# User-tian/Conan

Hardware: AMD Instinct MI355X
Metric: chunks/sec (80 ms chunk, 16 kHz), all streams summed; p50 per-chunk latency beside it (higher is better)
Workload: dtype f32 (3×bf16-limb products, f32 accumulate)

## Files before the change

### conan_amd/csrc/kernels.h

```cpp
#pragma once
#include <hip/hip_runtime.h>
#include <stdint.h>
#include <stdlib.h>

#include "voice_layout.h"

namespace cnk {

inline const char* dev_getenv(const char* name) {
#ifdef CONAN_DEV_SWITCHES
  return getenv(name);
#else
  (void)name;
  return nullptr;
#endif
}
#define HIP_CHECK(x) ::ch::hip_check((x), #x)


struct TRef {
  float* base;
  long long slot_stride;
  int C;
  int lmask;
// ... 101 lines not shown
  const int* tiles;
  const int* assign;
  int assign_per;
  int wr_max;
  float* slab; int* counters;
  long long slab_floats; int max_counters;
};
bool conv_limb_supported(const ConvArgs& a);
int conv_limb_shape(const ConvArgs* p, int nprob, int num_cu, int plan_n = 0, bool tail_split = false);
bool launch_conv_limb(const ConvLimbGroup& g, int shape, int num_cu, hipStream_t st);
int conv_limb_tail_slices(const ConvArgs& a, int shape, int num_cu);
const char* conv_limb_name(int shape);

struct RBProb {
  const float* w1; const float* w2;
  const float* b1; const float* b2;
  const unsigned short* w1l; const unsigned short* w2l;
  TRef x;
  TRef y;
  int k, dil;
};
struct RBArgs {
  RBProb p[3];
  const int* slots; const int* pos;
  const int* tiles;
  int ntiles;
  int* sched;
  int nprob, n, T;
  int tiles_per_slot;
  int order[3];
  float slope;
  int merge;
  TRef ymean;
  unsigned long long* dbg;
};
bool resblock_fused_supported(int C, int kmax, int span_max);
int resblock_fused_rows(int C, int T, int n, int ksum, int kmax, int num_cu);
bool launch_resblock_fused(const RBArgs& a, int C, int rows, int num_cu, hipStream_t st);
bool resblock_fused_can_merge(int C, int rows);
const char* resblock_fused_name(int C, int rows, bool merge = false);
const int* resblock_tiles(const RBArgs& a, int ro, int* total_out);
bool resblock_limb_supported(int C, int kmax, int span_max);
constexpr int kResblockLimbMaxSlots = 256;
int resblock_limb_rows(int C, int span_max);
bool launch_resblock_limb(const RBArgs& a, int C, int rows, int num_cu, hipStream_t st);
bool resblock_limb_can_merge(int C, int rows);
const char* resblock_limb_name(int C, int rows, bool merge = false);


struct RPProb {
  const float* w1; const float* w2;
  const float* b1; const float* b2;
  TRef x, y;
  TRef xh;
  int k, dil;
};
struct RPArgs {
  RPProb p[3];
  const int* slots; const int* pos;
  const int* tiles; int ntiles;
  int* sched;
  float* xb;
  unsigned* xflag; unsigned* mbox; unsigned* xcount;
  int nprob, n, T;
  float slope;
  unsigned* guard;
// ... 415 lines not shown
```

### conan_amd/csrc/resblock_limb.hip

```cpp
#include <algorithm>
#include <cstring>
#include <type_traits>

#include "kernels.h"

#define RL_MAX_SLOTS 256

#ifndef RL_HELPER_PRIO
#define RL_HELPER_PRIO 3
#endif
#ifndef RL_MATRIX_PRIO
#define RL_MATRIX_PRIO 0
#endif
#ifndef RL_STAMPS
#define RL_STAMPS 0
#endif

#ifdef RL_ABLATE_W
#define RL_WOFF(x) 0
#define RL_WOFF2(a_, b_) (b_)
#else
#define RL_WOFF(x) (x)
#define RL_WOFF2(a_, b_) (a_)
#endif

namespace cnk {

namespace {

typedef float f32x4 __attribute__((ext_vector_type(4)));
typedef __bf16 bf16x8 __attribute__((ext_vector_type(8)));
typedef unsigned short u16;
typedef const f32x4 __attribute__((address_space(1)))* gcf4;
typedef f32x4 __attribute__((address_space(1)))* gf4;
typedef const float __attribute__((address_space(1)))* gcf1;
typedef const int __attribute__((address_space(1)))* gci;

__device__ __forceinline__ f32x4 rl_gload(const void* p) { return *(gcf4)(p); }
__device__ __forceinline__ float4 rl_gload4(const float* p) { const f32x4 v = *(gcf4)(p); return make_float4(v[0], v[1], v[2], v[3]); }
__device__ __forceinline__ void rl_gstore4(float* p, const float4 v) { *(gf4)(p) = (f32x4){v.x, v.y, v.z, v.w}; }

typedef float f32x2 __attribute__((ext_vector_type(2)));
typedef __bf16 bf16x2 __attribute__((ext_vector_type(2)));
__device__ __forceinline__ void rl_split2(const f32x2 x, unsigned& h, unsigned& m, unsigned& l) {
  h = __builtin_bit_cast(unsigned, __builtin_convertvector(x, bf16x2));
  const f32x2 hf = {__uint_as_float(h << 16), __uint_as_float(h & 0xffff0000u)};
  const f32x2 r1 = x - hf;
  m = __builtin_bit_cast(unsigned, __builtin_convertvector(r1, bf16x2));
  const f32x2 mf = {__uint_as_float(m << 16), __uint_as_float(m & 0xffff0000u)};
  const f32x2 r2 = r1 - mf;
  l = __builtin_bit_cast(unsigned, __builtin_convertvector(r2, bf16x2));
}
__device__ __forceinline__ f32x2 rl_lrelu2(const f32x2 x, const float slope) {
  const f32x2 sx = x * slope;
  return (f32x2){__builtin_fmaxf(x[0], sx[0]), __builtin_fmaxf(x[1], sx[1])};
}

template <int C_, int NR2_, int SPAN_>
struct RLGeom {
  static constexpr int C = C_, NR2 = NR2_;
  static constexpr int NR1 = NR2 + 1;
  static constexpr int RO = 16 * NR2;
  static constexpr int XT_ROWS = 16 * NR1;
  static constexpr int MAXSPAN = SPAN_;
  static constexpr int WR_MAX = XT_ROWS + MAXSPAN;
  static constexpr int LDB = C + 16;
  static constexpr int PLW = WR_MAX * LDB;
  static constexpr int PLX = XT_ROWS * LDB;
  static constexpr int LDA = C + 4;
  static constexpr int LDS_U16 = 3 * (PLW + PLX);
  static constexpr int NCT = C / 16;
  static constexpr int NCW = C == 64 ? 1 : 2;
  static constexpr int RSPLIT = 4 / (NCT / NCW);
// ... 181 lines not shown
        const int idx = ht + 256 * u;
        const int w = idx / G::C4, c4 = idx - w * G::C4;
        const unsigned row = (rbase + (unsigned)w) & rmask;
        wv[u] = idx < wtotal ? rl_gload4(xb + (long long)row * C + c4 * 4) : make_float4(0.f, 0.f, 0.f, 0.f);
      }
      const long long abs0 = (xmode == 0 ? (long long)pos * xrate : 0ll) + t0 - (k - 1);
      wzr = abs0 >= 0 ? 0 : (abs0 < -(long long)G::XT_ROWS ? G::XT_ROWS : (int)-abs0);
    };
    auto win_write = [&]() __attribute__((always_inline)) {
#pragma unroll
      for (int u = 0; u < NIT; ++u) {
        const int idx = ht + 256 * u;
        const int w = idx / G::C4, c4 = idx - w * G::C4;
        unsigned h[2], m[2], l[2];
        rl_split2(rl_lrelu2((f32x2){wv[u].x, wv[u].y}, slope), h[0], m[0], l[0]);
        rl_split2(rl_lrelu2((f32x2){wv[u].z, wv[u].w}, slope), h[1], m[1], l[1]);
        if (idx < wtotal) {
          u16* dst = win + w * LDB + c4 * 4;
          *reinterpret_cast<uint2*>(dst) = make_uint2(h[0], h[1]);
          *reinterpret_cast<uint2*>(dst + G::PLW) = make_uint2(m[0], m[1]);
          *reinterpret_cast<uint2*>(dst + 2 * G::PLW) = make_uint2(l[0], l[1]);
        }
      }
      if (ht == 0) meta[0] = wzr;
    };
    constexpr int NOUT = (G::RO * G::C4) / 256;
    static_assert((G::RO * G::C4) % 256 == 0 && 256 % G::C4 == 0, "output tile / helper threads");
    const int oc4 = ht % G::C4;
    float4 oacc[NOUT], ores[NOUT], osum[MERGE ? NOUT : 1], ob2 = make_float4(0.f, 0.f, 0.f, 0.f);
    const float* oxb = nullptr; const float* ob2p = nullptr;
    float* oyb = nullptr;
    unsigned oyr0 = 0, oym = 0, oxr0 = 0, oxm = 0;
    int ot0 = 0, op = 0, oyC = C;
#pragma unroll
    for (int u = 0; u < (MERGE ? NOUT : 1); ++u) osum[u] = make_float4(0.f, 0.f, 0.f, 0.f);
    auto out_fetch = [&](const int p, const int i, const int t0, const int slot, const int pos) __attribute__((always_inline)) {
      const int xmode = a.p[0].x.mode, xrate = a.p[0].x.rate, ymode = a.p[0].y.mode, yrate = a.p[0].y.rate;
      oxb = RL_SEL(p, x.base) + (long long)(xmode == 0 ? slot : i) * RL_SEL(p, x.slot_stride);
      oxr0 = (xmode == 0 ? (unsigned)pos * (unsigned)xrate : 0u) + (unsigned)(RL_SEL(p, x.off) + t0);
      oxm = xmode == 0 ? (unsigned)RL_SEL(p, x.lmask) : 0xffffffffu;
      if (!merge) {
        oyb = RL_SEL(p, y.base) + (long long)(ymode == 0 ? slot : i) * RL_SEL(p, y.slot_stride);
        oyr0 = (ymode == 0 ? (unsigned)pos * (unsigned)yrate : 0u) + (unsigned)(RL_SEL(p, y.off) + t0);
        oym = ymode == 0 ? (unsigned)RL_SEL(p, y.lmask) : 0xffffffffu;
      } else {
        const int mmode = a.ymean.mode;
        oyb = a.ymean.base + (long long)(mmode == 0 ? slot : i) * a.ymean.slot_stride;
        oyr0 = (mmode == 0 ? (unsigned)pos * (unsigned)a.ymean.rate : 0u) + (unsigned)(a.ymean.off + t0);
        oym = mmode == 0 ? (unsigned)a.ymean.lmask : 0xffffffffu;
        oyC = a.ymean.C;
      }
      ot0 = t0; op = p;
      ob2p = RL_SEL(p, b2) + oc4 * 4;
#pragma unroll
      for (int u = 0; u < NOUT; ++u) oacc[u] = *reinterpret_cast<const float4*>(accimg + ((ht + 256 * u) / G::C4) * G::LDA + oc4 * 4);
      ob2 = rl_gload4(ob2p);
#pragma unroll
      for (int u = 0; u < NOUT; ++u) {
        const int r = (ht + 256 * u) / G::C4;
        ores[u] = ot0 + r < T ? rl_gload4(oxb + (long long)((oxr0 + (unsigned)r) & oxm) * C + oc4 * 4) : make_float4(0.f, 0.f, 0.f, 0.f);
      }
    };
    auto out_store = [&]() __attribute__((always_inline)) {
#pragma unroll
      for (int u = 0; u < NOUT; ++u) {
        const int r = (ht + 256 * u) / G::C4;
        if (ot0 + r < T) {
          const float4 v = make_float4((oacc[u].x + ob2.x) + ores[u].x, (oacc[u].y + ob2.y) + ores[u].y, (oacc[u].z + ob2.z) + ores[u].z, (oacc[u].w + ob2.w) + ores[u].w);
          if constexpr (!MERGE) rl_gstore4(oyb + (long long)((oyr0 + (unsigned)r) & oym) * C + oc4 * 4, v);
          else {
            float4 sm = osum[MERGE ? u : 0];
            if (op == 0) sm = v; else { sm.x += v.x; sm.y += v.y; sm.z += v.z; sm.w += v.w; }
            osum[MERGE ? u : 0] = sm;
            if (op == np - 1) {
              const float dn = (float)np;
              if (np > 1) { sm.x /= dn; sm.y /= dn; sm.z /= dn; sm.w /= dn; }
              sm.x = sm.x > 0.f ? sm.x : sm.x * slope; sm.y = sm.y > 0.f ? sm.y : sm.y * slope;
              sm.z = sm.z > 0.f ? sm.z : sm.z * slope; sm.w = sm.w > 0.f ? sm.w : sm.w * slope;
              rl_gstore4(oyb + (long long)((oyr0 + (unsigned)r) & oym) * oyC + oc4 * 4, sm);
            }
          }
        }
      }
    };
#if RL_STAMPS
    const unsigned long long h_t0 = __builtin_amdgcn_s_memtime();
    unsigned long long h_t[6] = {0, 0, 0, 0, 0, 0};
#define RL_HT(i_) h_t[i_] = __builtin_amdgcn_s_memtime() - h_t0
#else
#define RL_HT(i_)
#endif
    int dv0 = 0;
    if (wave == 4 && lane == 0) dv0 = __hip_atomic_fetch_add(a.sched, 1, __ATOMIC_RELAXED, __HIP_MEMORY_SCOPE_AGENT);
    for (int e = ht; e < a.n; e += 256) {
      const int sl = a.slots ? *(gci)(a.slots + e) : e;
      sptab[2 * e] = sl; sptab[2 * e + 1] = a.pos ? *(gci)(a.pos + sl) : 0;
    }
    const int tps = a.tiles_per_slot, per_prob = a.n * tps;
    auto decode = [&](const int e, int& p, int& i, int& t0) __attribute__((always_inline)) {
      if constexpr (!MERGE) {
        const int b = e / per_prob, rem = e - b * per_prob;
        p = b == 0 ? a.order[0] : (b == 1 ? a.order[1] : a.order[2]);
        i = rem / tps; t0 = (rem - i * tps) * G::RO;
      } else {
        const int g = e / np;
        p = e - g * np; i = g / tps; t0 = (g - i * tps) * G::RO;
      }
    };
    int cur = -1, p = -1, i = 0, t0 = 0;
    if (wave == 4) {
      cur = __builtin_amdgcn_readfirstlane(dv0) * (merge ? np : 1);
      if (cur >= ntiles) cur = -1;
      if (cur >= 0) decode(cur, p, i, t0);
      if (lane == 0) { meta[1] = cur; meta[2] = p; meta[3] = 0; }
    }
    RL_HT(0);
// ... 224 lines not shown
#endif
}


namespace {
struct RLCand { int C, NR2, span; };
const RLCand kLimbCands[] = {{32, 10, 50}, {64, 5, 50}, {128, 2, 50}};
}

bool resblock_limb_supported(int C, int kmax, int span_max) {
  for (const RLCand& c : kLimbCands)
    if (c.C == C && span_max <= c.span) return kmax <= 16;
  return false;
}

int resblock_limb_rows(int C, int span_max) {
  int best = 0;
  for (const RLCand& c : kLimbCands)
    if (c.C == C && span_max <= c.span) best = std::max(best, 16 * c.NR2);
  return best;
}

template <int C, int NR2, int SPAN, bool MERGE = false>
static bool launch_rl(const RBArgs& ain, int num_cu, hipStream_t st) {
  RBArgs a = ain;
  const int ro = 16 * NR2;
  a.tiles_per_slot = (a.T + ro - 1) / ro;
  const int total = a.nprob * a.n * a.tiles_per_slot;
  if (total <= 0) return true;
  if (!a.sched) return false;
  for (int p = 0; p < a.nprob; ++p) if (!a.p[p].w1l || !a.p[p].w2l) return false;
  if (a.n > RL_MAX_SLOTS) return false;
  if (!(a.slope > 0.f && a.slope <= 1.f)) return false;
  for (int p = 0; p < 3; ++p) a.order[p] = p;
  std::stable_sort(a.order, a.order + a.nprob, [&](int x, int y) { return a.p[x].k > a.p[y].k; });
  const int grid = std::min(a.merge ? total / a.nprob : total, num_cu);
  a.tiles = nullptr; a.ntiles = total;
  hipLaunchKernelGGL((resblock_limb_kernel<C, NR2, SPAN, MERGE>), dim3(grid), dim3(512), 0, st, a);
  return true;
}

bool launch_resblock_limb(const RBArgs& a, int C, int rows, int num_cu, hipStream_t st) {
  const int nr2 = rows / 16;
  if (a.merge) {
    if (C == 32 && nr2 == 10) return launch_rl<32, 10, 50, true>(a, num_cu, st);
    if (C == 64 && nr2 == 5) return launch_rl<64, 5, 50, true>(a, num_cu, st);
    if (C == 128 && nr2 == 2) return launch_rl<128, 2, 50, true>(a, num_cu, st);
    return false;
  }
  if (C == 32 && nr2 == 10) return launch_rl<32, 10, 50>(a, num_cu, st);
  if (C == 64 && nr2 == 5) return launch_rl<64, 5, 50>(a, num_cu, st);
  if (C == 128 && nr2 == 2) return launch_rl<128, 2, 50>(a, num_cu, st);
  return false;
}

bool resblock_limb_can_merge(int C, int rows) { return (C == 32 && rows == 160) || (C == 64 && rows == 80) || (C == 128 && rows == 32); }

const char* resblock_limb_name(int C, int rows, bool merge) {
  static thread_local char buf[72];
  const int span = 50;
  snprintf(buf, sizeof(buf), "cnk::resblock_limb_kernel<%d, %d, %d, %s>", C, rows / 16, span, merge ? "true" : "false");
  return buf;
}

}
```

### conan_amd/csrc/streams.h

```cpp
#pragma once
#include <array>
#include <functional>

#include "host_common.h"
#include "snapshot_layout.h"
#include "voice_layout.h"

using ch::Error;
using ch::Lin;
using ch::PackedConv;
using ch::Ring;
using cnk::ConvArgs;
using cnk::ConvGroup;
using cnk::TRef;

constexpr int kMaxBranches = 3;
constexpr int PADR = 16;

struct VocStage {
  Ring up;
  Ring upa;
  Ring xs;
  std::vector<std::vector<Ring>> xt, xo;
  std::vector<std::vector<Ring>> xa;
// ... 69 lines not shown
      auto it = dev_plan.find(name);
      if (it != dev_plan.end()) return it->second.c_str();
    }
#ifdef CONAN_DEV_SWITCHES
    return getenv((std::string("CONAN_") + name).c_str());
#else
    return nullptr;
#endif
  }
  bool fixed_plan = false;
  bool in_style_pass = false;
  int plan_n(int n) const { return (fixed_plan && !in_style_pass) ? max_slots : n; }
  bool pipe_idle = false;
  bool shared_device = false;
  int max_slots = 0, max_frames = 0, max_ref = 0, S_max = 0;
  std::vector<void*> allocs;
  int64_t state_bytes = 0;
  std::vector<std::pair<float*, long long>> voc_state, dec_state, emf_state;

  int* d_slots = nullptr;
  int* d_ident = nullptr;
  int* d_zero = nullptr;
  int* d_lens = nullptr;
  int* d_lens2 = nullptr;
  int* d_codes = nullptr;
  float* sk_slab[3] = {nullptr, nullptr, nullptr};
  int* sk_counters[3] = {nullptr, nullptr, nullptr};
  int reserve_cus = 0;
  bool fenced = false;
  bool rb_limb = false;
  bool arith_auto = true;
  bool rb_merge = true;
  int* cp_ticket[3] = {nullptr, nullptr, nullptr};
  int* rb_sched[2] = {nullptr, nullptr};
  float* rp_xb[2] = {nullptr, nullptr};
  unsigned* rp_words[2] = {nullptr, nullptr};
  long long sk_slab_floats = 0;
  int sk_max_tiles = 0;
  std::vector<int> h_slots;
  std::vector<int> slot_seen;
  int slot_gen = 0;
  PinRing pin;
  int* pos_emf = nullptr; int* pos_dec = nullptr; int* pos_voc = nullptr;
  unsigned* d_guard = nullptr;
  unsigned* h_guard = nullptr;
  int test_fault = 0;
  void check_fault() const {
    if (!h_guard) return;
    const unsigned code = *(volatile const unsigned*)h_guard;
    if (code == 0) return;
    static const char* what[] = {"?", "decoder_mega_kernel group / grid barrier", "emformer_fused_kernel cluster exchange", "resblock_pair_kernel partner flag", "resblock_pair_kernel tile mailbox",
                                 "(retired)", "decoder_mega_kernel xcd election", "decoder_mega_kernel xcd roll call", "decoder_mega_kernel xcd flag barrier"};
    throw ch::Error(CONAN_ERR_HIP, std::string("a cross-workgroup wait gave up after its 50 ms budget (") + what[code < 9 ? code : 0] +
                                       "): results since then are invalid and this stream-set is unusable - destroy it and create a new one");
  }

  struct FeSlot { long long recv = 0; int frames = 0, chunks = 0, phase = 0; };
  struct RsSlot { const ch::RsTable* f = nullptr; long long in = 0, out = 0; int phase = 0; };
  struct WavIn {
    float* fe_audio = nullptr; float* fe_mel = nullptr; float* fe_chunk = nullptr;
    int fe_LA = 0, fe_LM = 0, fe_last_n = 0;
    std::vector<FeSlot> fe_slot;
    StageSets<RgRow> rg_sets;
    int* rg_codes[kStageSets] = {}; float* rg_mel[kStageSets] = {}; float* rg_wav[kStageSets] = {};
    bool fe_last_ragged = false;
    std::vector<RsSlot> rs_slot;
// ... 129 lines not shown

  void mega_print_stamps();
  ~conan_streams() {
    if (live) live->fetch_sub(1);
    if (mega_dbg) mega_print_stamps();
    if (st_emf) (void)hipStreamDestroy(st_emf);
    if (st_front) (void)hipStreamDestroy(st_front);
    if (st_voc) (void)hipStreamDestroy(st_voc);
    for (int i = 0; i < NP; ++i) { if (ev_in[i]) (void)hipEventDestroy(ev_in[i]); if (ev_fence[i]) (void)hipEventDestroy(ev_fence[i]); }
    for (int i = 0; i < NP; ++i) { if (ev_wide[i]) (void)hipEventDestroy(ev_wide[i]); if (ev_emf[i]) (void)hipEventDestroy(ev_emf[i]); if (ev_front[i]) (void)hipEventDestroy(ev_front[i]); if (ev_voc[i]) (void)hipEventDestroy(ev_voc[i]); }
    for (void* p : allocs) (void)hipFree(p);
    if (h_guard) (void)hipHostFree(h_guard);
    for (auto& e : prof_ev) { (void)hipEventDestroy(e.first); (void)hipEventDestroy(e.second); }
    for (auto& e : clock_ev) (void)hipEventDestroy(e);
    for (auto& m : mega_cache) { if (m.copied) (void)hipEventDestroy(m.copied); if (m.pinned) (void)hipHostFree(m.pinned); if (m.dev) (void)hipFree(m.dev); }
    for (auto& e : tl_ev) (void)hipEventDestroy(e);
  }

  void build_vocoder();
  void build_emformer();
  void build_decoder();
  void set_slots(const int32_t* slots, int n, hipStream_t st);
  int pick_cfg(int M, int N, int nprob) const;
  bool prof_on = false;
  std::vector<std::pair<hipEvent_t, hipEvent_t>> prof_ev;
  size_t prof_used = 0;
  double prof_flops = 0.0;
  long long prof_launches = 0;
  struct ProfRec { std::string name; double flops; };
  std::vector<ProfRec> prof_rec;
  struct ProfKernel { std::string name; double ms, flops; long long n; };
  std::vector<ProfKernel> prof_kernels;
  void launch_group(const ConvGroup& g, int nprob, int cfg, hipStream_t st);
  bool launch_rb(const cnk::RBArgs& a, int C, hipStream_t st, const TRef* ymean = nullptr);
  void launch_rp(const cnk::RPArgs& a, hipStream_t st);
  bool use_rowconv = true;
  bool rowconv_ok(const PackedConv& pc, int dil, int T) const { return use_rowconv && pc.wf && cnk::rowconv_supported(pc.Cin, pc.k, dil, T); }
  cnk::RowConvArgs mk_rc(const PackedConv& pc, const TRef& x, const TRef& y, int n, int T, int dil = 1) const;
  void rowconv(const cnk::RowConvArgs& a, hipStream_t st);
  template <typename F> void profiled(const std::string& name, double flops, hipStream_t st, F&& launch);
  void conv(const ConvArgs& a, hipStream_t st) { ConvGroup g; g.p[0] = a; launch_group(g, 1, pick_cfg(plan_n(a.n) * a.T, a.Cout, 1), st); }
  ConvArgs mk(const PackedConv& pc, const TRef& x, const TRef& y, int n, int T, const int* pos, int dil = 1, int pad_left = -1) const;

  struct DecExtra { float* mel_out2 = nullptr; int* codes_dst = nullptr; const int* codes_src = nullptr; int codes_words = 0;
                    const float* f0_in = nullptr; const float* uv_in = nullptr; };
  struct MegaProgram {
    long long key[8] = {0, 0, 0, 0, 0, 0, 0, 0};
    bool ok = false;
    int nops = 0, groups = 0, group_size = 0, njobs = 0, kw4 = 0, lds_bytes = 0, barriers = 0, n = 0, T = 0;
    int lds_need = 0;
    bool xcd = false;
    double flops = 0.0;
    cnk::MegaOp* dev = nullptr;
    cnk::MegaOp* pinned = nullptr;
    hipEvent_t copied = nullptr;
    long long stamp = 0;
  };
  static constexpr int kMegaMaxOps = cnk::kMegaMaxOps, kMegaEntries = 12;
  std::vector<MegaProgram> mega_cache;
  long long mega_clock = 0;
  bool use_mega = true;
  int mega_grid = 128;
  int mega_gs = 8;
  bool mega_narrow_ksplit = true;
  int mega_ffn_gs = 8;
  unsigned* mega_bar = nullptr;
  unsigned mega_bar_count = 0;
// ... 107 lines not shown
```

### conan_amd/csrc/streams.hip

```cpp
#include <climits>

#include "streams.h"


ConvArgs conan_streams::mk(const PackedConv& pc, const TRef& x, const TRef& y, int n, int T, const int* pos, int dil,
                           int pad_left) const {
  ConvArgs a;
  memset(&a, 0, sizeof(a));
  a.x = x;
  a.y = y; a.res = ch::null_ref(); a.m1 = ch::null_ref(); a.m2 = ch::null_ref();
  a.w = pc.w; a.bias = pc.bias; a.bvec = nullptr; a.slots = d_slots; a.pos = pos; a.lens = nullptr;
  a.Cin = pc.Cin; a.Cin_pad = pc.Cin_pad; a.Cin_alloc = pc.Cin_alloc; a.Cout = pc.Cout; a.Cout_pad = pc.Cout_pad;
  a.ktaps = pc.k; a.dil = dil; a.pad_left = pad_left < 0 ? (pc.k - 1) * dil : pad_left;
  a.T = T; a.n = n; a.in_act = cnk::ACT_NONE; a.in_slope = 0.f; a.out_act = cnk::ACT_NONE; a.out_scale = 1.f; a.out_slope = 0.f;
  a.shuffle_r = pc.shuffle_r;
  a.wl = reinterpret_cast<const unsigned short*>(pc.wl);
  if (x.C != pc.Cin && !(x.C > pc.Cin)) throw Error(CONAN_ERR_SHAPE, "conv input width mismatch");
  return a;
}

int conan_streams::pick_cfg(int M, int N, int nprob) const {
  const int wide[] = {cnk::CFG_64x64, cnk::CFG_32x64_K2, cnk::CFG_32x32_K4};
  const int narrow[] = {cnk::CFG_128x32, cnk::CFG_64x32_K2, cnk::CFG_32x32_K4};
  const int* order = N <= 32 ? narrow : wide;
// ... 112 lines not shown
void conan_streams::rowconv(const cnk::RowConvArgs& a, hipStream_t st) {
  const double fl = 2.0 * (double)a.n * a.T * a.Cout * a.ktaps * a.Cin;
  if (mega_rec) {
    cnk::MegaOp op; memset(&op, 0, sizeof(op));
    op.u.rc = a;
    int ldsf = 0;
    const int prows = fixed_plan ? plan_n(a.n) * a.T : 0;
    const int v = cnk::rowconv_plan(op.u.rc, &op.nbx, &op.nby, &ldsf, prows);
    op.type = v == 3 ? cnk::MOP_ROWLIN : (v == 2 ? cnk::MOP_RC114 : cnk::MOP_RC111);
    const int strips64 = (op.u.rc.Cout_pad + 63) / 64;
    if (v == 0 && !a.w2 && plan_n(a.n) * a.T > 16 && mega_narrow_ksplit && (strips64 * 4 <= mega_gs || (strips64 * 2 <= mega_gs && a.ktaps >= 3)) && (a.ktaps * (a.Cin >> 4)) % 4 == 0) {
      const int ldsk = (32 + op.u.rc.wr_max * (a.Cin + 8) + 3 * 64 * 4);
      cnk::MegaOp t = op; t.type = cnk::MOP_RC114;
      if (cnk::decoder_mega_lds_floats(t, ldsk) * 4 <= (96 + 32 * 264) * 4) {
        op.type = cnk::MOP_RC114; op.nbx = (op.u.rc.Cout_pad + 15) / 16; ldsf = ldsk;
      }
    }
    if (a.w2) {
      if ((v != 0 && v != 2) || (a.ktaps * (a.Cin >> 4)) % 8 != 0) { mega_rec_ok = false; return; }
      op.type = cnk::MOP_FFN;
      const int hc = a.Cout / mega_ffn_gs;
      op.u.rc.hid_overlay = hc == 64 ? 1 : 0;
      ldsf = op.u.rc.hid_overlay ? std::max(op.u.rc.wr_max * (a.Cin + 8), 16 * (hc + 8)) : op.u.rc.wr_max * (a.Cin + 8) + 16 * (hc + 8);
      mega_rec_flops += 2.0 * (double)a.n * a.T * a.Cout * a.Cout2;
    }
    mega_rec_flops += fl;
    mega_push(op, cnk::decoder_mega_lds_floats(op, ldsf));
    return;
  }
  const int prows = fixed_plan ? plan_n(a.n) * a.T : 0;
  profiled(cnk::rowconv_kernel_name(a, prows), fl, st, [&] { cnk::launch_rowconv(a, st, prows); });
}

bool conan_streams::launch_rb(const cnk::RBArgs& ain, int C, hipStream_t st, const TRef* ymean) {
  cnk::RBArgs a = ain;
  a.sched = rb_sched[ws_index(st) == 1 ? 1 : 0];
  int ksum = 0, kmax = 0;
  double fl = 0.0;
  for (int p = 0; p < a.nprob; ++p) { ksum += a.p[p].k; kmax = std::max(kmax, a.p[p].k); fl += 2.0 * 2.0 * (double)a.n * a.T * C * C * a.p[p].k; }
  const int cus = std::max(8, ctx->num_cu - (ws_index(st) == 1 ? reserve_cus : 0));
  int span = 0;
  bool limb = rb_limb;
  for (int p = 0; p < a.nprob; ++p) { span = std::max(span, (a.p[p].k - 1) * a.p[p].dil); limb = limb && a.p[p].w1l && a.p[p].w2l; }
  limb = limb && plan_n(a.n) <= cnk::kResblockLimbMaxSlots && cnk::resblock_limb_supported(C, kmax, span);
  const int rows = limb ? cnk::resblock_limb_rows(C, span) : cnk::resblock_fused_rows(C, a.T, plan_n(a.n), ksum, kmax, cus);
  const long long groups = (long long)plan_n(a.n) * ((a.T + rows - 1) / rows);
  const long long rounds = (groups + cus - 1) / cus;
  const bool balanced = groups * 10 >= rounds * cus * 9;
  a.merge = (ymean && rb_merge && a.nprob > 1 && groups >= cus && balanced && (limb ? cnk::resblock_limb_can_merge(C, rows) : cnk::resblock_fused_can_merge(C, rows))) ? 1 : 0;
  if (a.merge) a.ymean = *ymean;
  profiled(limb ? cnk::resblock_limb_name(C, rows, a.merge != 0) : cnk::resblock_fused_name(C, rows, a.merge != 0), fl, st, [&] {
    if (!(limb ? cnk::launch_resblock_limb(a, C, rows, cus, st) : cnk::launch_resblock_fused(a, C, rows, cus, st))) throw Error(CONAN_ERR_HIP, "fused resblock launch failed");
  });
  return a.merge != 0;
}

void conan_streams::launch_rp(const cnk::RPArgs& ain, hipStream_t st) {
  cnk::RPArgs a = ain;
  const int w = ws_index(st) == 1 ? 1 : 0;
  const int pairs = ctx->num_cu / 2;
  a.xb = rp_xb[w]; a.xflag = rp_words[w]; a.mbox = rp_words[w] + (size_t)pairs * 8; a.xcount = rp_words[w] + (size_t)pairs * 12;
  a.sched = reinterpret_cast<int*>(rp_words[w] + (size_t)pairs * 14);
  a.guard = d_guard; a.fault = test_fault == 3 ? 1 : 0;
  if (test_fault == 3) test_fault = 0;
  double fl = 0.0;
  for (int p = 0; p < a.nprob; ++p) fl += 2.0 * 2.0 * (double)a.n * a.T * 256.0 * 256.0 * a.p[p].k;
  profiled(cnk::resblock_pair_name(a.T), fl, st, [&] {
    if (!cnk::launch_resblock_pair(a, ctx->num_cu, st)) throw Error(CONAN_ERR_HIP, "resblock pair launch failed");
  });
}

void conan_streams::mega_print_stamps() {
  if (!mega_dbg || mega_dbg_prog < 0 || mega_dbg_prog >= (int)mega_cache.size()) return;
  (void)hipDeviceSynchronize();
  const MegaProgram& e = mega_cache[mega_dbg_prog];
  std::vector<unsigned long long> h(cnk::kMegaDbgWords);
  if (hipMemcpy(h.data(), mega_dbg, h.size() * 8, hipMemcpyDeviceToHost) != hipSuccess) return;
  static const char* names[] = {"rowconv<1,1,1>", "rowconv<1,1,4>", "rowlin", "layernorm", "xattn", "pitch_head", "embed", "copy32", "advance", "ffn"};
  constexpr int nnames = (int)(sizeof(names) / sizeof(names[0]));
  fprintf(stderr, "[decoder_mega] last launch: %d groups x %d workgroups, %d jobs, %d operators, %d group barriers, %.1f us in all (workgroup 0; first job per operator below)\n",
          e.groups, e.group_size, e.njobs, e.nops, e.barriers, (h[e.nops + 1] - h[0]) / 100.0);
  if (!e.xcd) {
    fprintf(stderr, "  groups on one XCD (l2 mode) / XCC masks:");
    for (int g2 = 0; g2 < e.groups && g2 < 32; ++g2) if (h[cnk::kMegaDbgGroupWords + g2]) fprintf(stderr, " %d:%llu/%02llx", g2, h[cnk::kMegaDbgGroupWords + g2] & 1ull, (h[cnk::kMegaDbgGroupWords + g2] >> 16) & 0xffull);
    fprintf(stderr, "\n");
  }
  for (int o = 0; o < e.nops; ++o) {
// ... 13 lines not shown
  if (stamps && !mega_dbg) mega_dbg = reinterpret_cast<unsigned long long*>(alloc(2 * (size_t)cnk::kMegaDbgWords));
  if (stamps) HIP_CHECK(hipMemsetAsync(mega_dbg, 0, sizeof(unsigned long long) * cnk::kMegaDbgWords, st));
  if (stamps) mega_dbg_prog = (int)(&e - mega_cache.data());
  cnk::MegaLaunch m; memset(&m, 0, sizeof(m));
  m.prog = e.dev; m.nops = e.nops; m.njobs = e.njobs; m.groups = e.groups; m.group_size = e.group_size; m.kw4 = e.kw4; m.lds_bytes = e.lds_bytes;
  m.slots = d_slots; m.pos = pos_dec; m.n = e.n; m.T = e.T;
  m.gbar = mega_bar + 16; m.bar = mega_bar; m.bar_base = mega_bar_count; m.dbg = mega_dbg; m.guard = d_guard; m.wide_regs = rb_limb ? 1 : 0;
  m.xcd = e.xcd ? 1 : 0;
  const bool pipelined = st_front != nullptr && st == st_front;
  if (e.xcd) {
    static const bool pad_always = ch::dev_getenv("CONAN_MEGA_XCD_PAD") != nullptr;
    if (pipelined && !pad_always) m.lds_bytes = e.lds_need;
    mega_xseq = mega_xseq + 1u;
    m.xs = mega_x; m.xseq = mega_xseq; m.xdec_base = mega_xdec;
    if (test_fault == 1) { m.xseq += 7u; mega_xseq += 7u; test_fault = 0; }
    profiled("cnk::decoder_mega_kernel<4, 2>", e.flops, st, [&] { cnk::launch_decoder_mega(m, st); });
    mega_xdec += (unsigned)(e.groups * e.group_size);
    return;
  }
  if (test_fault == 1) { m.bar_base += 1u; test_fault = 0; }
  mega_gseq = mega_gseq + 1u;
  m.xs = mega_x; m.xseq = mega_gseq;
  { const bool nol2 = dev("MEGA_NOL2") != nullptr;
    const char* lay = dev("MEGA_LAYOUT");
    const bool mfast = lay && lay[0] == 'm';
    m.xdec_base = (nol2 ? 1u : 0u) | (mfast ? 2u : 0u); }
  profiled(rb_limb ? "cnk::decoder_mega_kernel<4, 3>" : "cnk::decoder_mega_kernel<6, 3>", e.flops, st, [&] { cnk::launch_decoder_mega(m, st); });
  mega_bar_count += (unsigned)(e.groups * e.group_size);
}

void conan_streams::parse_dev_plan(const char* text) {
  static const char* known[] = {"RESERVE_CUS", "ROWCONV", "RB_NOMERGE", "RB_NOLIMB", "FENCED", "DEC_MEGA", "MEGA_GRID", "FRONT_CUSTRIDE", "EMF_CUSTRIDE", "MEGA_GS",
                                "MEGA_NARROW", "MEGA_NOL2", "MEGA_LAYOUT", "FRONT_PRIO", "RB_UNFUSED", "RB_FUSED", "RB_PAIR", "RB_NOPAIR", "RP_MIN_SLOTS",
                                "UPS_CFG", "EMF_CLUSTER", "EMF_UNFUSED", "NO_TALL", "TALL_MAXT"};
  dev_plan.clear();
  if (!text) return;
  const std::string t(text);
  size_t p = 0;
  while (p < t.size()) {
    size_t q = t.find(';', p);
    if (q == std::string::npos) q = t.size();
    std::string item = t.substr(p, q - p);
    p = q + 1;
    while (!item.empty() && item.front() == ' ') item.erase(item.begin());
    while (!item.empty() && item.back() == ' ') item.pop_back();
    if (item.empty()) continue;
    const size_t eq = item.find('=');
    const std::string name = item.substr(0, eq), value = eq == std::string::npos ? "1" : item.substr(eq + 1);
    bool ok = false;
    for (const char* k : known) ok = ok || name == k;
    if (!ok) throw Error(CONAN_ERR_INVALID, "conan_streams_opts.dev_plan: unknown switch '" + name + "'");
    dev_plan[name] = value;
  }
}

void conan_streams::set_slots(const int32_t* slots, int n, hipStream_t st) {
  if (n <= 0 || n > max_slots) throw Error(CONAN_ERR_INVALID, "slot count out of range");
  bool same = (int)h_slots.size() == n;
  for (int i = 0; i < n; ++i) {
    if (slots[i] < 0 || slots[i] >= max_slots) throw Error(CONAN_ERR_INVALID, "slot index out of range");
    if (same && h_slots[i] != slots[i]) same = false;
  }
  if (same) return;
  if (++slot_gen == 0x7fffffff) { std::fill(slot_seen.begin(), slot_seen.end(), 0); slot_gen = 1; }
  for (int i = 0; i < n; ++i) {
    if (slot_seen[slots[i]] == slot_gen) throw Error(CONAN_ERR_INVALID, "duplicate slot");
    slot_seen[slots[i]] = slot_gen;
// ... 71 lines not shown
        c.voc_num_resblocks <= kMaxBranches && max_slots >= (dev("RP_MIN_SLOTS") ? atoi(dev("RP_MIN_SLOTS")) : 16) && max_frames * rate <= 32) {
      s.pair = true;
      for (int b = 0; b < c.voc_num_resblocks; ++b)
        for (int d = 0; d < c.voc_rb_num_dil; ++d)
          s.pair = s.pair && cnk::resblock_pair_supported(ch_, c.voc_rb_kernels[b], (c.voc_rb_kernels[b] - 1) * c.voc_rb_dilations[b][d], max_frames * rate);
      s.fused = s.pair;
    }
    int up_hist = (maxk - 1) * c.voc_rb_dilations[0][0];
    if (s.fused) for (int b = 0; b < c.voc_num_resblocks; ++b) up_hist = std::max(up_hist, (c.voc_rb_kernels[b] - 1) * (c.voc_rb_dilations[b][0] + 1));
    s.up = mk_ring(ch_, rate, up_hist, &voc_state);
    const int next_pad = (i + 1 < c.voc_num_ups) ? c.voc_up_kernels[i + 1] - 1 : 6;
    s.xs = mk_ring(ch_, rate, next_pad, &voc_state);
    if (!s.fused) s.upa = mk_ring(ch_, rate, (maxk - 1) * c.voc_rb_dilations[0][0], &voc_state);
    s.xt.resize(c.voc_num_resblocks); s.xo.resize(c.voc_num_resblocks); s.xa.resize(c.voc_num_resblocks);
    for (int b = 0; b < c.voc_num_resblocks; ++b)
      for (int d = 0; d < c.voc_rb_num_dil; ++d) {
        const int k = c.voc_rb_kernels[b];
        if (!s.fused) s.xt[b].push_back(mk_ring(ch_, rate, k - 1, &voc_state));
        const int h = (d + 1 < c.voc_rb_num_dil) ? (k - 1) * (c.voc_rb_dilations[b][d + 1] + (s.fused ? 1 : 0)) : next_pad;
        s.xo[b].push_back(mk_ring(ch_, rate, h, &voc_state));
        if (!s.fused && d + 1 < c.voc_rb_num_dil) s.xa[b].push_back(mk_ring(ch_, rate, h, &voc_state));
      }
    if (s.pair) {
      s.xh.resize(c.voc_num_resblocks);
      for (int b = 0; b < c.voc_num_resblocks; ++b)
        for (int d = 0; d < c.voc_rb_num_dil; ++d) s.xh[b].push_back(mk_ring(ch_, rate, c.voc_rb_kernels[b] - 1, &voc_state));
      for (int w = 0; w < 2 && !rp_xb[w]; ++w) {
        const int pairs = ctx->num_cu / 2;
        rp_xb[w] = alloc(cnk::resblock_pair_xb_floats(ctx->num_cu));
        rp_words[w] = reinterpret_cast<unsigned*>(alloc((size_t)pairs * 14 + 4));
      }
    }
  }
}

void conan_streams::hifigan_step(int n, int frames, const float* mel_dev, float* wav_out_dev, float* pre_tanh, hipStream_t st, const conan_hifigan_taps* taps,
                                 const OutPlan* op) {
  const conan_cfg& c = ctx->cfg;
  const int* pos = pos_voc;
  const float LR = 0.1f;
  const bool lookahead = c.voc_upsample == 2;
  for (int i = 0; i < n; ++i) {
    if (lookahead && !voc_fresh[h_slots[i]])
      throw Error(CONAN_ERR_STATE, "upsample 'nn' (CausalUpsampleBlock1) looks ahead of the frame it writes: slot " + std::to_string(h_slots[i]) +
                                       " needs conan_streams_reset(CONAN_MODEL_HIFIGAN) before every vocoder step (whole-utterance or windowed forward only)");
    voc_fresh[h_slots[i]] = 0;
  }
  const bool out_rows = op && op->active;
  int oq = -1;
  if (out_rows) {
    out_stage_init();
    oq = wav_out.or_sets.begin(op->rows.data(), n, st);
  }
  {
    cnk::CopyArgs ca; memset(&ca, 0, sizeof(ca));
    ca.x = ch::lin_ref(const_cast<float*>(mel_dev), frames, c.num_mels); ca.y = v_mel.ref();
    ca.slots = d_slots; ca.pos = pos; ca.lens = nullptr; ca.T = frames; ca.n = n; ca.C = c.num_mels;
    cnk::launch_copy_rows(ca, st);
  }
  {
    ConvArgs a = mk(ctx->conv("voc.conv_pre"), v_mel.ref(), v_pre.ref(), n, frames, pos);
    a.out_act = cnk::ACT_LRELU; a.out_slope = LR;
    conv(a, st);
  }
  auto tap = [&](float* dst, const Ring& r, int T) {
    if (!dst) return;
    cnk::CopyArgs ca; memset(&ca, 0, sizeof(ca));
    ca.x = r.ref(); ca.y = ch::lin_ref(dst, T, r.C); ca.slots = d_slots; ca.pos = pos; ca.T = T; ca.n = n; ca.C = r.C;
    cnk::launch_copy_rows(ca, st);
  };
  if (taps) tap(taps->conv_pre_act, v_pre, frames);
  const int NB = c.voc_num_resblocks, ND = c.voc_rb_num_dil;
  if (NB > kMaxBranches) throw Error(CONAN_ERR_UNSUPPORTED, "more than 3 resblock branches");
  int ridx = 0;
  bool last_merged = false;
  for (int i = 0; i < c.voc_num_ups; ++i) {
    VocStage& s = v_st[i];
    bool merged = false;
    const int Tin = frames * (s.rate / c.voc_up_rates[i]);
    const int T = frames * s.rate;
    {
      ConvArgs a = mk(ctx->conv("voc.ups." + std::to_string(i)), i == 0 ? v_pre.ref() : v_st[i - 1].xs.ref(), s.up.ref(), n, Tin, pos, 1,
                      lookahead ? 0 : -1);
      if (!s.fused) { a.y2_base = s.upa.base; a.y2_slope = LR; }
      {
        const std::vector<int> forced = [&] { std::vector<int> v; const char* e = dev("UPS_CFG"); if (e) { std::string t(e); size_t p = 0; while (p <= t.size()) { size_t q = t.find(',', p); if (q == std::string::npos) q = t.size(); v.push_back(atoi(t.substr(p, q - p).c_str())); p = q + 1; } } return v; }();
        if (i < (int)forced.size() && forced[i] >= 0 && forced[i] < cnk::NUM_CFG) { ConvGroup g; g.p[0] = a; launch_group(g, 1, forced[i], st); }
        else conv(a, st);
      }
      if (taps) tap(taps->ups[i], s.up, T);
    }
    for (int d = 0; d < ND && s.pair; ++d) {
      if (T > 32) throw Error(CONAN_ERR_INVALID, "more frames in a step than this stream-set was created for");
      cnk::RPArgs ra; memset(&ra, 0, sizeof(ra));
      for (int b = 0; b < NB; ++b) {
        const std::string base = "voc.rbf." + std::to_string(ridx + b);
        cnk::RPProb& pr = ra.p[b];
        pr.w1 = ctx->vec(base + ".c1." + std::to_string(d) + ".w"); pr.b1 = ctx->vec(base + ".c1." + std::to_string(d) + ".b");
        pr.w2 = ctx->vec(base + ".c2." + std::to_string(d) + ".w"); pr.b2 = ctx->vec(base + ".c2." + std::to_string(d) + ".b");
        pr.x = d == 0 ? s.up.ref() : s.xo[b][d - 1].ref();
        pr.y = s.xo[b][d].ref();
        pr.xh = s.xh[b][d].ref();
        pr.k = c.voc_rb_kernels[b]; pr.dil = c.voc_rb_dilations[b][d];
      }
      ra.slots = d_slots; ra.pos = pos; ra.nprob = NB; ra.n = n; ra.T = T; ra.slope = LR;
      launch_rp(ra, st);
      if (d + 1 == ND && mark_wide) { HIP_CHECK(hipEventRecord(mark_wide, st)); for (int q = 0; q < 4; ++q) if (ev_wide[q] == mark_wide) wide_marked[q] = true; }
    }
    for (int d = 0; d < ND && s.fused && !s.pair; ++d) {
      cnk::RBArgs ra; memset(&ra, 0, sizeof(ra));
      for (int b = 0; b < NB; ++b) {
        const std::string base = "voc.rbf." + std::to_string(ridx + b);
        cnk::RBProb& pr = ra.p[b];
        pr.w1 = ctx->vec(base + ".c1." + std::to_string(d) + ".w"); pr.b1 = ctx->vec(base + ".c1." + std::to_string(d) + ".b");
        pr.w2 = ctx->vec(base + ".c2." + std::to_string(d) + ".w"); pr.b2 = ctx->vec(base + ".c2." + std::to_string(d) + ".b");
        pr.w1l = reinterpret_cast<const unsigned short*>(ctx->vec_or_null(base + ".c1." + std::to_string(d) + ".wl"));
        pr.w2l = reinterpret_cast<const unsigned short*>(ctx->vec_or_null(base + ".c2." + std::to_string(d) + ".wl"));
        pr.x = d == 0 ? s.up.ref() : s.xo[b][d - 1].ref();
        pr.y = s.xo[b][d].ref();
        pr.k = c.voc_rb_kernels[b]; pr.dil = c.voc_rb_dilations[b][d];
      }
      ra.slots = d_slots; ra.pos = pos; ra.nprob = NB; ra.n = n; ra.T = T; ra.slope = LR;
      if (d + 1 < ND) launch_rb(ra, s.C, st);
      else { const TRef ym = s.xs.ref(); merged = launch_rb(ra, s.C, st, &ym); }
    }
    for (int d = 0; d < ND && c.voc_resblock == 2; ++d) {
      ConvGroup g1;
      for (int b = 0; b < NB; ++b) {
        const TRef xin = d == 0 ? s.up.ref() : s.xo[b][d - 1].ref();
        const TRef xin_act = d == 0 ? s.upa.ref() : s.xa[b][d - 1].ref();
        ConvArgs a1 = mk(ctx->conv("voc.rb." + std::to_string(ridx + b) + ".c." + std::to_string(d)), xin_act, s.xo[b][d].ref(), n, T, pos,
                         c.voc_rb_dilations[b][d]);
        a1.res = xin; a1.has_res = 1;
        if (d + 1 < ND) { a1.y2_base = s.xa[b][d].base; a1.y2_slope = LR; }
        g1.p[b] = a1;
      }
      launch_group(g1, NB, pick_cfg(plan_n(n) * T, s.C, NB), st);
    }
    for (int d = 0; d < ND && c.voc_resblock != 2 && !s.fused; ++d) {
      ConvGroup g1, g2;
      for (int b = 0; b < NB; ++b) {
        const TRef xin = d == 0 ? s.up.ref() : s.xo[b][d - 1].ref();
        const TRef xin_act = d == 0 ? s.upa.ref() : s.xa[b][d - 1].ref();
        std::string base = "voc.rb." + std::to_string(ridx + b);
        ConvArgs a1 = mk(ctx->conv(base + ".c1." + std::to_string(d)), xin_act, s.xt[b][d].ref(), n, T, pos, c.voc_rb_dilations[b][d]);
        a1.out_act = cnk::ACT_LRELU; a1.out_slope = LR;
        g1.p[b] = a1;
        ConvArgs a2 = mk(ctx->conv(base + ".c2." + std::to_string(d)), s.xt[b][d].ref(), s.xo[b][d].ref(), n, T, pos, 1);
        a2.res = xin; a2.has_res = 1;
        if (d + 1 < ND) { a2.y2_base = s.xa[b][d].base; a2.y2_slope = LR; }
        g2.p[b] = a2;
      }
      const int cfg = pick_cfg(plan_n(n) * T, s.C, NB);
      launch_group(g1, NB, cfg, st);
      launch_group(g2, NB, cfg, st);
    }
    const bool tap_last = taps && taps->stage_out[i] && i + 1 == c.voc_num_ups && !merged;
    last_merged = merged || tap_last;
    if ((i + 1 < c.voc_num_ups || tap_last) && !merged) {
      cnk::MeanActArgs ma; memset(&ma, 0, sizeof(ma));
      for (int b = 0; b < NB; ++b) ma.x[b] = s.xo[b][ND - 1].ref();
      ma.y = s.xs.ref(); ma.slots = d_slots; ma.pos = pos; ma.nsrc = NB; ma.T = T; ma.n = n; ma.C = s.C; ma.slope = LR;
      cnk::launch_mean_act(ma, st);
    }
    if (taps) tap(taps->stage_out[i], s.xs, T);
    ridx += NB;
  }
  {
    VocStage& s = v_st.back();
    const int T = frames * s.rate;
    cnk::ConvPostArgs a; memset(&a, 0, sizeof(a));
    if (last_merged) { a.x[0] = s.xs.ref(); a.nsrc = 1; }
    else { for (int b = 0; b < NB; ++b) a.x[b] = s.xo[b][ND - 1].ref(); a.nsrc = NB; a.xmean = s.xs.ref(); }
    a.slope = LR;
    a.w = ctx->vec("voc.conv_post.w"); a.bias = ctx->scalars.at("voc.conv_post.b");
    a.wav = out_rows ? wav_out.or_wav[oq] : wav_out_dev; a.pre = pre_tanh; a.slots = d_slots; a.pos = pos; a.T = T; a.n = n; a.C = s.C; a.k = (int)ctx->scalars.at("voc.conv_post.k");
    a.adv_pos = pos_voc; a.adv_delta = frames; a.adv_ticket = cp_ticket[ws_index(st)];
    cnk::launch_conv_post(a, st);
    if (out_rows) resample_out(*op, oq, T, st);
    if (!op || op->dst.empty()) wav_out.out_counts.assign(n, T);
    for (int i = 0; i < n; ++i) {
      const int slot = h_slots[i];
      wav_out.voc_samples[slot] += T;
      if (!op) continue;
      if (!wav_out.or_slot.empty() && wav_out.or_slot[slot].f && out_rows) wav_out.or_slot[slot].out += op->counts[i];
      wav_out.out_counts[op->dst.empty() ? i : op->dst[i]] = op->counts[i];
    }
  }
}


void conan_streams::build_emformer() {
  const conan_cfg& c = ctx->cfg;
  const int D = c.emf_input_dim, Q = c.emf_segment + c.emf_right_context;
  for (int l = 0; l < c.emf_layers; ++l) {
    Ring r; r.C = D; r.rate = 1; r.L = ch::next_pow2(c.emf_left_context + c.emf_segment); r.slot_stride = (long long)r.L * D;
// ... 194 lines not shown
```

Baseline: 47330.

## Fuse resblock mean-activation into limb kernel via per-tile atomic tickets

When the final dilation's resblock launch isn't merged, each output wave now stores its branch result with an sc1 store, then bumps a per-tile atomic counter. The last of the three branches to finish reads all three outputs back, averages them, applies leaky ReLU and writes the stage mean. This is meant to remove the separate mean_act kernel launch and its full re-read of the three branch outputs. In exchange it adds atomics, a vmcnt wait and extra loads on the tail wave, plus inline asm with cache-scope bits that depends on memory-ordering assumptions.

After: 47490 (median of 6 runs). Within noise of the previous version (+0.3%).

```diff
diff --git a/conan_amd/csrc/kernels.h b/conan_amd/csrc/kernels.h
--- a/conan_amd/csrc/kernels.h
+++ b/conan_amd/csrc/kernels.h
@@ -157,6 +157,8 @@
   float slope;
   int merge;
   TRef ymean;
+  int tmean; int* tickets;
+  int tshift;
   unsigned long long* dbg;
 };
 bool resblock_fused_supported(int C, int kmax, int span_max);
diff --git a/conan_amd/csrc/resblock_limb.hip b/conan_amd/csrc/resblock_limb.hip
--- a/conan_amd/csrc/resblock_limb.hip
+++ b/conan_amd/csrc/resblock_limb.hip
@@ -39,6 +39,17 @@
 __device__ __forceinline__ f32x4 rl_gload(const void* p) { return *(gcf4)(p); }
 __device__ __forceinline__ float4 rl_gload4(const float* p) { const f32x4 v = *(gcf4)(p); return make_float4(v[0], v[1], v[2], v[3]); }
 __device__ __forceinline__ void rl_gstore4(float* p, const float4 v) { *(gf4)(p) = (f32x4){v.x, v.y, v.z, v.w}; }
+
+__device__ __forceinline__ void rl_xstore4(float* p, const float4 v) {
+  const f32x4 d = {v.x, v.y, v.z, v.w};
+  asm volatile("global_store_dwordx4 %0, %1, off sc1\n\ts_nop 1" ::"v"(p), "v"(d) : "memory");
+}
+__device__ __forceinline__ void rl_xload4x3(const float* b0, const float* b1, const float* b2, int byte_off, float4& v0, float4& v1, float4& v2) {
+  f32x4 d0, d1, d2;
+  asm volatile("s_nop 4\n\tglobal_load_dwordx4 %0, %3, %4 sc1\n\tglobal_load_dwordx4 %1, %3, %5 sc1\n\tglobal_load_dwordx4 %2, %3, %6 sc1\n\ts_waitcnt vmcnt(0)"
+               : "=&v"(d0), "=&v"(d1), "=&v"(d2) : "v"(byte_off), "s"(b0), "s"(b1), "s"(b2) : "memory");
+  v0 = make_float4(d0[0], d0[1], d0[2], d0[3]); v1 = make_float4(d1[0], d1[1], d1[2], d1[3]); v2 = make_float4(d2[0], d2[1], d2[2], d2[3]);
+}
 
 typedef float f32x2 __attribute__((ext_vector_type(2)));
 typedef __bf16 bf16x2 __attribute__((ext_vector_type(2)));
@@ -286,6 +297,12 @@
     float* oyb = nullptr;
     unsigned oyr0 = 0, oym = 0, oxr0 = 0, oxm = 0;
     int ot0 = 0, op = 0, oyC = C;
+    typedef const RBArgs __attribute__((address_space(4)))* kargs_t;
+    auto kargs = [&]() __attribute__((always_inline)) {
+      kargs_t k = (kargs_t)__builtin_amdgcn_kernarg_segment_ptr();
+      asm volatile("" : "+s"(k));
+      return k;
+    };
 #pragma unroll
     for (int u = 0; u < (MERGE ? NOUT : 1); ++u) osum[u] = make_float4(0.f, 0.f, 0.f, 0.f);
     auto out_fetch = [&](const int p, const int i, const int t0, const int slot, const int pos) __attribute__((always_inline)) {
@@ -315,14 +332,50 @@
         ores[u] = ot0 + r < T ? rl_gload4(oxb + (long long)((oxr0 + (unsigned)r) & oxm) * C + oc4 * 4) : make_float4(0.f, 0.f, 0.f, 0.f);
       }
     };
+    auto mean_store = [&]() __attribute__((always_inline)) {
+      if constexpr (!MERGE) {
+        asm volatile("s_waitcnt vmcnt(0)" ::: "memory");
+        const kargs_t ka = kargs();
+        const long long sd = oyb - (op == 0 ? ka->p[0].y.base : (op == 1 ? ka->p[1].y.base : ka->p[2].y.base));
+        int* const ctr = ka->tickets + ((sd >> ka->tshift) * ka->tiles_per_slot + ot0 / G::RO) * 4 + (wave - 4);
+        int ticket = 0;
+        if (lane == 0) ticket = __hip_atomic_fetch_add(ctr, 1, __ATOMIC_RELAXED, __HIP_MEMORY_SCOPE_AGENT);
+        ticket = __builtin_amdgcn_readfirstlane(ticket);
+        if (ticket != np - 1) return;
+        if (lane == 0) __hip_atomic_store(ctr, 0, __ATOMIC_RELAXED, __HIP_MEMORY_SCOPE_AGENT);
+        const float* const s0 = ka->p[0].y.base + sd; const float* const s1 = ka->p[1].y.base + sd; const float* const s2 = ka->p[2].y.base + sd;
+        float* const mb = ka->ymean.base + sd;
+        const float dn = (float)np;
+#pragma unroll 1
+        for (int u = 0; u < NOUT; ++u) {
+          const int r = (ht + 256 * u) / G::C4;
+          if (ot0 + r < T) {
+            const int ro = (int)((oyr0 + (unsigned)r) & oym) * C + oc4 * 4;
+            float4 v, v1, v2;
+            rl_xload4x3(s0, s1, s2, ro * 4, v, v1, v2);
+            v.x += v1.x; v.y += v1.y; v.z += v1.z; v.w += v1.w;
+            v.x += v2.x; v.y += v2.y; v.z += v2.z; v.w += v2.w;
+            v.x /= dn; v.y /= dn; v.z /= dn; v.w /= dn;
+            v.x = v.x > 0.f ? v.x : v.x * slope; v.y = v.y > 0.f ? v.y : v.y * slope;
+            v.z = v.z > 0.f ? v.z : v.z * slope; v.w = v.w > 0.f ? v.w : v.w * slope;
+            rl_gstore4(mb + ro, v);
+          }
+        }
+      }
+    };
     auto out_store = [&]() __attribute__((always_inline)) {
+      bool tmean = false;
+      if constexpr (!MERGE) tmean = kargs()->tmean != 0;
 #pragma unroll
       for (int u = 0; u < NOUT; ++u) {
         const int r = (ht + 256 * u) / G::C4;
         if (ot0 + r < T) {
           const float4 v = make_float4((oacc[u].x + ob2.x) + ores[u].x, (oacc[u].y + ob2.y) + ores[u].y, (oacc[u].z + ob2.z) + ores[u].z, (oacc[u].w + ob2.w) + ores[u].w);
-          if constexpr (!MERGE) rl_gstore4(oyb + (long long)((oyr0 + (unsigned)r) & oym) * C + oc4 * 4, v);
-          else {
+          if constexpr (!MERGE) {
+            float* const yp = oyb + (long long)((oyr0 + (unsigned)r) & oym) * C + oc4 * 4;
+            if (tmean) rl_xstore4(yp, v);
+            else rl_gstore4(yp, v);
+          } else {
             float4 sm = osum[MERGE ? u : 0];
             if (op == 0) sm = v; else { sm.x += v.x; sm.y += v.y; sm.z += v.z; sm.w += v.w; }
             osum[MERGE ? u : 0] = sm;
@@ -336,6 +389,7 @@
           }
         }
       }
+      if (tmean) mean_store();
     };
 #if RL_STAMPS
     const unsigned long long h_t0 = __builtin_amdgcn_s_memtime();
@@ -626,6 +680,16 @@
   for (int p = 0; p < a.nprob; ++p) if (!a.p[p].w1l || !a.p[p].w2l) return false;
   if (a.n > RL_MAX_SLOTS) return false;
   if (!(a.slope > 0.f && a.slope <= 1.f)) return false;
+  if (a.tmean) {
+    if (MERGE || a.merge || a.nprob != 3 || !a.tickets || !a.ymean.base) return false;
+    const long long ss = a.p[0].y.slot_stride;
+    if (ss <= 0 || (ss & (ss - 1)) != 0) return false;
+    a.tshift = 0;
+    while ((1ll << a.tshift) < ss) ++a.tshift;
+    auto same = [](const TRef& x, const TRef& y) { return x.mode == y.mode && x.slot_stride == y.slot_stride && x.C == y.C && x.lmask == y.lmask && x.rate == y.rate && x.off == y.off; };
+    for (int p = 0; p < 3; ++p)
+      if (a.p[p].y.mode != 0 || a.p[p].y.C != C || !same(a.p[p].y, a.p[0].y) || !same(a.p[p].y, a.ymean) || ((long long)a.p[p].y.lmask + 1) * C * 4 >= (1ll << 31)) return false;
+  }
   for (int p = 0; p < 3; ++p) a.order[p] = p;
   std::stable_sort(a.order, a.order + a.nprob, [&](int x, int y) { return a.p[x].k > a.p[y].k; });
   const int grid = std::min(a.merge ? total / a.nprob : total, num_cu);
diff --git a/conan_amd/csrc/streams.h b/conan_amd/csrc/streams.h
--- a/conan_amd/csrc/streams.h
+++ b/conan_amd/csrc/streams.h
@@ -125,6 +125,9 @@
   bool arith_auto = true;
   bool rb_merge = true;
   int* cp_ticket[3] = {nullptr, nullptr, nullptr};
+  int* tm_tickets[3] = {nullptr, nullptr, nullptr};
+  long long tm_max_units = 0;
+  bool ticket_mean = false;
   int* rb_sched[2] = {nullptr, nullptr};
   float* rp_xb[2] = {nullptr, nullptr};
   unsigned* rp_words[2] = {nullptr, nullptr};
@@ -320,7 +323,7 @@
   struct ProfKernel { std::string name; double ms, flops; long long n; };
   std::vector<ProfKernel> prof_kernels;
   void launch_group(const ConvGroup& g, int nprob, int cfg, hipStream_t st);
-  bool launch_rb(const cnk::RBArgs& a, int C, hipStream_t st, const TRef* ymean = nullptr);
+  bool launch_rb(const cnk::RBArgs& a, int C, hipStream_t st, const TRef* ymean = nullptr, bool ticket_ok = false);
   void launch_rp(const cnk::RPArgs& a, hipStream_t st);
   bool use_rowconv = true;
   bool rowconv_ok(const PackedConv& pc, int dil, int T) const { return use_rowconv && pc.wf && cnk::rowconv_supported(pc.Cin, pc.k, dil, T); }
diff --git a/conan_amd/csrc/streams.hip b/conan_amd/csrc/streams.hip
--- a/conan_amd/csrc/streams.hip
+++ b/conan_amd/csrc/streams.hip
@@ -168,7 +168,7 @@
   profiled(cnk::rowconv_kernel_name(a, prows), fl, st, [&] { cnk::launch_rowconv(a, st, prows); });
 }
 
-bool conan_streams::launch_rb(const cnk::RBArgs& ain, int C, hipStream_t st, const TRef* ymean) {
+bool conan_streams::launch_rb(const cnk::RBArgs& ain, int C, hipStream_t st, const TRef* ymean, bool ticket_ok) {
   cnk::RBArgs a = ain;
   a.sched = rb_sched[ws_index(st) == 1 ? 1 : 0];
   int ksum = 0, kmax = 0;
@@ -185,10 +185,17 @@
   const bool balanced = groups * 10 >= rounds * cus * 9;
   a.merge = (ymean && rb_merge && a.nprob > 1 && groups >= cus && balanced && (limb ? cnk::resblock_limb_can_merge(C, rows) : cnk::resblock_fused_can_merge(C, rows))) ? 1 : 0;
   if (a.merge) a.ymean = *ymean;
+  if (!a.merge && ymean && ticket_ok && ticket_mean && limb && a.nprob == 3 && ymean->mode == 0) {
+    auto same = [](const TRef& x, const TRef& y) { return x.mode == y.mode && x.slot_stride == y.slot_stride && x.C == y.C && x.lmask == y.lmask && x.rate == y.rate && x.off == y.off; };
+    const long long units = (long long)max_slots * ((a.T + rows - 1) / rows) * 4, ss = ymean->slot_stride;
+    bool tm = units <= tm_max_units && ss > 0 && (ss & (ss - 1)) == 0 && ymean->C == C;
+    for (int p = 0; p < 3; ++p) tm = tm && same(a.p[p].y, *ymean);
+    if (tm) { a.tmean = 1; a.tickets = tm_tickets[ws_index(st)]; a.ymean = *ymean; }
+  }
   profiled(limb ? cnk::resblock_limb_name(C, rows, a.merge != 0) : cnk::resblock_fused_name(C, rows, a.merge != 0), fl, st, [&] {
     if (!(limb ? cnk::launch_resblock_limb(a, C, rows, cus, st) : cnk::launch_resblock_fused(a, C, rows, cus, st))) throw Error(CONAN_ERR_HIP, "fused resblock launch failed");
   });
-  return a.merge != 0;
+  return a.merge != 0 || a.tmean != 0;
 }
 
 void conan_streams::launch_rp(const cnk::RPArgs& ain, hipStream_t st) {
@@ -268,7 +275,7 @@
 void conan_streams::parse_dev_plan(const char* text) {
   static const char* known[] = {"RESERVE_CUS", "ROWCONV", "RB_NOMERGE", "RB_NOLIMB", "FENCED", "DEC_MEGA", "MEGA_GRID", "FRONT_CUSTRIDE", "EMF_CUSTRIDE", "MEGA_GS",
                                 "MEGA_NARROW", "MEGA_NOL2", "MEGA_LAYOUT", "FRONT_PRIO", "RB_UNFUSED", "RB_FUSED", "RB_PAIR", "RB_NOPAIR", "RP_MIN_SLOTS",
-                                "UPS_CFG", "EMF_CLUSTER", "EMF_UNFUSED", "NO_TALL", "TALL_MAXT"};
+                                "UPS_CFG", "EMF_CLUSTER", "EMF_UNFUSED", "NO_TALL", "TALL_MAXT", "NO_TICKET_MEAN"};
   dev_plan.clear();
   if (!text) return;
   const std::string t(text);
@@ -406,6 +413,23 @@
       }
     }
   }
+  ticket_mean = rb_limb && max_slots >= 16 && c.voc_num_resblocks == 3 && dev("NO_TICKET_MEAN") == nullptr;
+  if (ticket_mean) {
+    long long units = 0;
+    for (int i = 0; i + 1 < c.voc_num_ups; ++i) {
+      const VocStage& s = v_st[i];
+      const long long T = (long long)max_frames * s.rate;
+      if (s.fused && !s.pair) {
+        int span = 0;
+        for (int b = 0; b < c.voc_num_resblocks; ++b) span = std::max(span, (c.voc_rb_kernels[b] - 1) * c.voc_rb_dilations[b][c.voc_rb_num_dil - 1]);
+        const int rows = cnk::resblock_limb_rows(s.C, span);
+        if (rows > 0) units = std::max(units, (long long)max_slots * ((T + rows - 1) / rows) * 4);
+      }
+    }
+    tm_max_units = units;
+    for (int w = 0; w < 3 && units > 0; ++w) tm_tickets[w] = (int*)alloc((size_t)units);
+    if (units == 0) ticket_mean = false;
+  }
 }
 
 void conan_streams::hifigan_step(int n, int frames, const float* mel_dev, float* wav_out_dev, float* pre_tanh, hipStream_t st, const conan_hifigan_taps* taps,
@@ -451,6 +475,7 @@
   for (int i = 0; i < c.voc_num_ups; ++i) {
     VocStage& s = v_st[i];
     bool merged = false;
+    const bool mean_ticket_ok = i + 1 < c.voc_num_ups && !(taps && taps->stage_out[i]);
     const int Tin = frames * (s.rate / c.voc_up_rates[i]);
     const int T = frames * s.rate;
     {
@@ -496,7 +521,7 @@
       }
       ra.slots = d_slots; ra.pos = pos; ra.nprob = NB; ra.n = n; ra.T = T; ra.slope = LR;
       if (d + 1 < ND) launch_rb(ra, s.C, st);
-      else { const TRef ym = s.xs.ref(); merged = launch_rb(ra, s.C, st, &ym); }
+      else { const TRef ym = s.xs.ref(); merged = launch_rb(ra, s.C, st, &ym, mean_ticket_ok); }
     }
     for (int d = 0; d < ND && c.voc_resblock == 2; ++d) {
       ConvGroup g1;
@@ -535,7 +560,7 @@
       cnk::MeanActArgs ma; memset(&ma, 0, sizeof(ma));
       for (int b = 0; b < NB; ++b) ma.x[b] = s.xo[b][ND - 1].ref();
       ma.y = s.xs.ref(); ma.slots = d_slots; ma.pos = pos; ma.nsrc = NB; ma.T = T; ma.n = n; ma.C = s.C; ma.slope = LR;
-      cnk::launch_mean_act(ma, st);
+      profiled("cnk::mean_act_kernel", 0.0, st, [&] { cnk::launch_mean_act(ma, st); });
     }
     if (taps) tap(taps->stage_out[i], s.xs, T);
     ridx += NB;
```
